# AlvinYH/Faster-VoxelPose

Hardware: AMD Instinct MI355X
Metric: frames/sec at 5-view 80x80x20 voxel (heatmaps -> 3D joints); MPJPE vs ref (mm) in mpjpe_vs_ref_mm (higher is better)
Workload: dtype f32

## Files before the change

### faster-voxelpose_amd/csrc/fvp_conv_wino.hip

```cpp
#include <hip/hip_runtime.h>

#include <algorithm>
#include <cstdio>
#include <type_traits>

#include "fvp_conv_args.h"

#ifndef FVP_WINO_ABLATE
#define FVP_WINO_ABLATE 0
#endif

namespace fvp {

typedef float f32x4 __attribute__((ext_vector_type(4)));

template <int N>
__device__ __forceinline__ void wait_vmcnt_imm() {
  static_assert(N >= 0 && N < 64, "vmcnt");
  __builtin_amdgcn_s_waitcnt(0x0f70 | (N & 15) | ((N >> 4) << 14));
}

constexpr unsigned kWinoOOB = 0x80000000u;

template <int WC, int WT, int CC, int NI, bool HAS_RES, bool RESW, int CW = 2>
__global__ void __launch_bounds__(WC * WT * 64, (WC * WT == 16 ? 4 : 2)) k_conv_wino(ConvArgs a) {
  HIP_DYNAMIC_SHARED(float, smem)
  constexpr int NWV = WC * WT;
  constexpr int NT = NWV * 64;
  static_assert(NWV == 16 || NWV == 8 || NWV == 4, "4, 8 or 16 waves");
  static_assert(CW == 1 || CW == 2, "cout blocks per wave");
  static_assert(CC == 4 || CC == 8, "chunk");
  static_assert(NI >= 1 && NI <= 4, "input DMA rounds");
  constexpr int CBW = 16 * CW * WC;
  constexpr int WCH = CC * CBW * 16;
  constexpr int WS_SZ = RESW ? 0 : WCH;
  constexpr int NW = RESW ? 0 : CC * CBW * 4 / NT;
  static_assert(RESW || (CC * CBW * 4) % NT == 0, "whole weight DMA rounds");
  constexpr int NPS = NI + NW;
  constexpr int S = CC / 4;
  constexpr int XS_SZ = NI * NT * 4;
  constexpr int BUF_SZ = XS_SZ + WS_SZ;
  constexpr bool kDiag = FVP_WINO_ABLATE != 0;
  const int t = threadIdx.x, lane = t & 63;
  const int wave = __builtin_amdgcn_readfirstlane(t >> 6);
  const int k4 = lane >> 4, l15 = lane & 15;
  const int wc = wave % WC, wt = wave / WC;
  const int W = a.W, THp = a.TH + 2, WP = W + 4;
  const int plane_sz = THp * WP;
  const int CS = a.TN * plane_sz;
  const int ablate = kDiag ? a.ablate : 0;
  const bool dma = !(ablate & 1);

  const int epi_off = 4 + 3 * BUF_SZ + (RESW ? a.cinp * CBW * 16 : 0);
  const unsigned char* const vflag = reinterpret_cast<const unsigned char*>(smem + epi_off + 3 * a.coutp);

  const int G = gridDim.x, nunits = a.nunits;
  auto next_unit = [&](int u, auto from_lds) {
    if (a.nflags > 0) {
      while (u < nunits) {
        const int pg = fdiv_nb(fdiv_nb(u, a.m_ys), a.m_ty);
        const int f = fdiv_nb(pg, a.m_vd);
        const int ok = decltype(from_lds)::value ? int(vflag[f]) : int(a.plane_valid[f]);
        if (__builtin_amdgcn_readfirstlane(ok)) break;
        u += G;
      }
    }
    return u;
  };
  using LdsFlags = std::integral_constant<bool, true>;
  using GlobalFlags = std::integral_constant<bool, false>;
  int u = next_unit(int(blockIdx.x), GlobalFlags{});
  if (u >= nunits) return;

  const int q0 = wt * 16 + l15;
  int poff;
  {
    const bool q_ok = q0 < a.TN * a.tpp;
    const int q = q_ok ? q0 : 0;
    const int tn = fdiv_nb(q, a.m_tpp), trem = q - tn * a.tpp;
    const int ty = fdiv_nb(trem, a.m_tpr), tx = trem - ty * a.tpr;
    poff = tn * plane_sz + 2 * ty * WP + 3 + 2 * tx + k4 * CS;
  }
  const int swz = (l15 >> 2) & 3;
  const int a0 = (k4 * CBW + wc * (16 * CW) + l15) * 16 + swz * 4;
  int aoff[4];
#pragma unroll
  for (int xi = 0; xi < 4; ++xi) aoff[xi] = a0 ^ (xi << 2);
  const float* const wres = smem + 4 + 3 * BUF_SZ;
  auto wchunk = [&](const float* slot, int k) { return RESW ? wres + k * WCH : slot + XS_SZ; };

  f32x4 acc[CW][16];

  const int HW = a.H * W;
  const int nchunks = a.cinp / CC;

  unsigned voff[NI];
  auto item_pos = [&](int j, int& ry, int& n, bool& inside, int& ci, int& qd) {
    const int qpr = (W >> 2) + 1;
    const int rows_per_ch = a.TN * THp;
    const int nin = CC * rows_per_ch * qpr + 1;
    int ln = lane;
    FVP_OPAQUE_V(ln);
    const int it = (wave + NWV * j) * 64 + ln;
    const int row = fdiv_nb(it, a.m_qpr);
    qd = it - row * qpr;
    ci = fdiv_nb(row, a.m_rpc);
    const int rem = row - ci * rows_per_ch;
    n = fdiv_nb(rem, a.m_thp);
    ry = rem - n * THp;
    inside = it < nin && qd > 0 && ci < CC;
  };
#pragma unroll
  for (int j = 0; j < NI; ++j) {
    int ry, n, ci, qd;
    bool inside;
    item_pos(j, ry, n, inside, ci, qd);
    voff[j] = inside ? unsigned((n * a.cin + ci) * HW + ry * W + 4 * (qd - 1)) * 4u : 0u;
    __builtin_amdgcn_sched_barrier(0);
  }
  constexpr int DCI = NT / (CBW * 4);
  const unsigned woffb = (unsigned(t / (CBW * 4)) * unsigned(a.coutp) * 16u + 4u * unsigned(t % (CBW * 4))) * 4u;
  const unsigned wdj4 = unsigned(DCI) * unsigned(a.coutp) * 64u;
  const unsigned in_step4 = unsigned(CC) * unsigned(HW) * 4u;
  const unsigned w_step4 = unsigned(CC) * unsigned(a.coutp) * 64u;
  const unsigned lds0 = FVP_LDS_BYTE_ADDRESS(smem) + 16u + unsigned(wave) * 1024u;
  i32x4 rs_in = {0, 0, 0x7ffffff0, 0x00020000}, rs_w = {0, 0, 0x7ffffff0, 0x00020000};
  auto set_base = [](i32x4& rs, const float* p) {
    const unsigned long long b = reinterpret_cast<unsigned long long>(p);
    rs[0] = __builtin_amdgcn_readfirstlane(int(unsigned(b)));
    rs[1] = __builtin_amdgcn_readfirstlane(int(unsigned(b >> 32) & 0xffffu));
  };
  int su = u, sk = 0;
  auto enter_unit = [&](int su_) {
    const KArgsPtr ka = FVP_FRESH_ARGS(a);
    const int ys = ka->ysplit, tys = ka->tiles_y;
    const int st = fdiv_nb(su_, ka->m_ys), sy = su_ - st * ys;
    const int spg = fdiv_nb(st, ka->m_ty), sty = st - spg * tys;
    const int splane0 = spg * ka->TN, sy0 = sty * ka->TH;
    const int H = ka->H, planes = ka->planes;
    set_base(rs_in, ka->src + size_t(splane0) * ka->cin * HW + sy0 * W - W);
    set_base(rs_w, ka->wts + size_t(sy) * (CBW * 16));
#pragma unroll
    for (int j = 0; j < NI; ++j) {
      int ry, n, ci, qd;
      bool inside;
      item_pos(j, ry, n, inside, ci, qd);
      const bool ok = inside && unsigned(sy0 + ry - 1) < unsigned(H) && splane0 + n < planes;
      voff[j] = (voff[j] & 0x7fffffffu) | (ok ? 0u : kWinoOOB);
      __builtin_amdgcn_sched_barrier(0);
    }
  };
  auto stage = [&](int k, int slot) {
    const unsigned la0 = lds0 + unsigned(slot) * unsigned(BUF_SZ * 4);
    const unsigned so_in = unsigned(k) * in_step4;
#pragma unroll
    for (int j = 0; j < NI; ++j) asm_buffer_load_lds16(la0 + unsigned(NWV * j) * 1024u, voff[j], rs_in, so_in);
    const unsigned so_w = unsigned(k) * w_step4;
#pragma unroll
    for (int j = 0; j < NW; ++j)
      asm_buffer_load_lds16(la0 + unsigned(XS_SZ * 4 + NWV * j * 1024), woffb, rs_w, so_w + unsigned(j) * wdj4);
  };
  enter_unit(su);
  auto stage_next = [&](int slot, auto from_lds) {
    if (su >= nunits) return false;
    stage(sk, slot);
    if (++sk == nchunks) {
      sk = 0;
      su = next_unit(su + G, from_lds);
      if (su < nunits) enter_unit(su);
    }
    return true;
  };

  float4 av[CW][4];
  float d[4][4];
  float v[4][4];
  auto fetch_a = [&](int cb, const float* wbase, int s) {
    if (kDiag && (ablate & 256)) return;
    int a0o = a0;
    if (CW == 1) FVP_OPAQUE_V(a0o);
#pragma unroll
    for (int xi = 0; xi < 4; ++xi)
      av[cb][xi] = *reinterpret_cast<const float4*>(wbase + (CW == 1 ? (a0o ^ (xi << 2)) : aoff[xi]) + (s * 4 * CBW * 16 + cb * 256));
  };
  auto fetch_d = [&](const float* base, int s, int wp) {
    const float* xs = base + poff + s * 4 * CS;
#pragma unroll
    for (int r = 0; r < 4; ++r) {
      const float* row = xs + r * wp;
      const float2 m = *reinterpret_cast<const float2*>(row + 1);
      d[r][0] = row[0];
      d[r][1] = m.x;
      d[r][2] = m.y;
      d[r][3] = row[3];
    }
  };
  auto transform = [&](float (&tr)[4][4]) {
#pragma unroll
    for (int c = 0; c < 4; ++c) {
      tr[0][c] = d[0][c] - d[2][c];
      tr[1][c] = d[1][c] + d[2][c];
      tr[2][c] = d[2][c] - d[1][c];
      tr[3][c] = d[1][c] - d[3][c];
    }
  };
  auto columns = [&](const float (&tr)[4][4]) {
#pragma unroll
    for (int xi = 0; xi < 4; ++xi) {
      v[xi][0] = tr[xi][0] - tr[xi][2];
      v[xi][1] = tr[xi][1] + tr[xi][2];
      v[xi][2] = tr[xi][2] - tr[xi][1];
      v[xi][3] = tr[xi][1] - tr[xi][3];
    }
  };
  auto mfma16 = [&](int cb, auto firstc) {
    if (kDiag && (ablate & 4)) return;
    const f32x4 z = {0.0f, 0.0f, 0.0f, 0.0f};
#pragma unroll
    for (int xi = 0; xi < 4; ++xi) {
      const float aw[4] = {av[cb][xi].x, av[cb][xi].y, av[cb][xi].z, av[cb][xi].w};
#pragma unroll
      for (int nu = 0; nu < 4; ++nu)
        acc[cb][4 * xi + nu] = __builtin_amdgcn_mfma_f32_16x16x4f32(
            aw[nu], v[xi][nu], decltype(firstc)::value ? z : acc[cb][4 * xi + nu], 0, 0, 0);
    }
  };

  if (RESW) {
    const int rounds = (a.cinp * CBW * 4) / NT;
    for (int j = 0; j < rounds; ++j)
      asm_global_load_lds16(a.wts + size_t((wave + NWV * j) * 64 + lane) * 4,
                            __builtin_amdgcn_readfirstlane(FVP_LDS_BYTE_ADDRESS(smem) +
                                                           4u * unsigned(4 + 3 * BUF_SZ + (wave + NWV * j) * 256)));
  }
  {
    float* const e = const_cast<float*>(smem) + epi_off;
    for (int i = t; i < 3 * a.coutp; i += NT) e[i] = a.epi[i];
    unsigned char* const f = const_cast<unsigned char*>(vflag);
    for (int i = t; i < a.nflags; i += NT) f[i] = a.plane_valid[i];
  }
  if (dma) {
    stage_next(0, GlobalFlags{});
    stage_next(1, GlobalFlags{});
  }
  wait_vmcnt_imm<0>();
  __syncthreads();

  int cur = 0;
  auto slot_ptr = [&](int slot) { return smem + 4 + slot * BUF_SZ; };
  fetch_a(0, wchunk(slot_ptr(0), 0), 0);
  fetch_d(slot_ptr(0), 0, WP);
  while (true) {
    auto chunk = [&](int k, auto firstc) {
      constexpr bool kFirst = decltype(firstc)::value;
      const int nxt = cur == 2 ? 0 : cur + 1;
      const int nn = nxt == 2 ? 0 : nxt + 1;
      const bool more = dma && stage_next(nn, LdsFlags{});
      const float* const cs = slot_ptr(cur);
      const float* const ns = slot_ptr(nxt);
      int wp = WP;
      FVP_OPAQUE(wp);
      if constexpr (CW == 2) {
#pragma unroll
      for (int s = 0; s < S; ++s) {
        __builtin_amdgcn_s_waitcnt(0xc07f);
        __builtin_amdgcn_sched_barrier(0);
        fetch_a(1, wchunk(cs, k), s);
        __builtin_amdgcn_sched_barrier(0);
        float tr[4][4];
        if (kDiag && (ablate & 512)) {
#pragma unroll
          for (int r = 0; r < 4; ++r)
#pragma unroll
            for (int c = 0; c < 4; ++c) v[r][c] = d[r][c];
        } else {
          transform(tr);
        }
        if (s + 1 < S) fetch_d(cs, s + 1, wp);
        __builtin_amdgcn_sched_barrier(0);
        if (!(kDiag && (ablate & 512))) columns(tr);
        if (kFirst && s == 0) mfma16(0, std::integral_constant<bool, true>{});
        else mfma16(0, std::integral_constant<bool, false>{});
        __builtin_amdgcn_sched_barrier(0);
        __builtin_amdgcn_s_waitcnt(0xc07f);
        __builtin_amdgcn_sched_barrier(0);
        if (s + 1 < S) {
          fetch_a(0, wchunk(cs, k), s + 1);
        } else {
          if (!kFirst && dma) {
            if (more) wait_vmcnt_imm<NPS>();
            else wait_vmcnt_imm<0>();
          }
          if (!(kDiag && (ablate & 128))) __builtin_amdgcn_s_barrier();
          if (k + 1 < nchunks) {
            fetch_a(0, wchunk(ns, k + 1), 0);
            fetch_d(ns, 0, wp);
          }
        }
        __builtin_amdgcn_sched_barrier(0);
        if (kFirst && s == 0) mfma16(1, std::integral_constant<bool, true>{});
        else mfma16(1, std::integral_constant<bool, false>{});
        __builtin_amdgcn_sched_barrier(0);
      }
      } else {
#pragma unroll
        for (int s = 0; s < S; ++s) {
          __builtin_amdgcn_s_waitcnt(0xc07f);
          __builtin_amdgcn_sched_barrier(0);
          {
            float tr[4][4];
            transform(tr);
            columns(tr);
          }
          __builtin_amdgcn_sched_barrier(0);
          if (kFirst && s == 0) mfma16(0, std::integral_constant<bool, true>{});
          else mfma16(0, std::integral_constant<bool, false>{});
          __builtin_amdgcn_sched_barrier(0);
          if (s + 1 < S) {
            fetch_a(0, wchunk(cs, k), s + 1);
            fetch_d(cs, s + 1, wp);
          } else {
            if (!kFirst && dma) {
              if (more) wait_vmcnt_imm<NPS>();
              else wait_vmcnt_imm<0>();
            }
            __builtin_amdgcn_s_barrier();
            if (k + 1 < nchunks) {
              fetch_a(0, wchunk(ns, k + 1), 0);
              fetch_d(ns, 0, wp);
            }
          }
          __builtin_amdgcn_sched_barrier(0);
        }
      }
      cur = nxt;
    };
    chunk(0, std::integral_constant<bool, true>{});
    for (int k = 1; k < nchunks; ++k) chunk(k, std::integral_constant<bool, false>{});

    if (!(ablate & 8)) {
      const KArgsPtr ka = FVP_FRESH_ARGS(a);
      const int ys = ka->ysplit, tys = ka->tiles_y;
      const int ut = fdiv_nb(u, ka->m_ys), uy = u - ut * ys;
      const int pg = fdiv_nb(ut, ka->m_ty), ty_i = ut - pg * tys;
      const int plane0 = pg * ka->TN, y0 = ty_i * ka->TH, co0 = uy * CBW;
      const int cout = ka->cout, coutp = ka->coutp;
      const int flags = ka->flags;
      float* const dst = ka->dst;
      const float* const res = ka->res;
      float* const pool_dst = ka->pool_dst;
      int le = lane;
      FVP_OPAQUE_V(le);
      const int k4 = le >> 4;
      const int qe = wt * 16 + (le & 15);
      const bool q_ok = qe < ka->TN * ka->tpp;
      const int qq = q_ok ? qe : 0;
      const int tn = fdiv_nb(qq, ka->m_tpp), trem = qq - tn * ka->tpp;
      const int ty = fdiv_nb(trem, ka->m_tpr), tx = trem - ty * ka->tpr;
      const bool relu = flags & FVP_EPI_RELU;
      const bool res_after = flags & FVP_EPI_RES_AFTER_RELU;
      const int plane = plane0 + tn, y = y0 + 2 * ty, x = 2 * tx;
      const bool tile_ok = q_ok && plane < ka->planes && y < ka->H;
      const unsigned ppix = unsigned((y >> 1) * (W >> 1) + tx);
      const float* const epi_s = smem + epi_off;
      const bool fast = relu && !res_after;
      unsigned HW4 = unsigned(HW) * 4u, W4 = unsigned(W) * 4u, HWq4 = unsigned(HW >> 2) * 4u;
      FVP_OPAQUE(HW4);
      FVP_OPAQUE(W4);
      FVP_OPAQUE(HWq4);
      i32x4 rs = {0, 0, 0x7ffffff0, 0x00020000};
      if (HAS_RES) set_base(rs, res + size_t(plane0) * cout * HW);
      const unsigned lco = unsigned(tn * cout + co0 + wc * (16 * CW) + 4 * k4);
      const unsigned omask = (kDiag && (ablate & 1024)) ? 0x3ffffu : 0x7fffffffu;
      const unsigned voff0 = tile_ok ? ((lco * unsigned(HW) + unsigned(y * W + x)) * 4u) & omask : kWinoOOB;
      const unsigned voffp = tile_ok ? (lco * unsigned(HW >> 2) + ppix) * 4u : kWinoOOB;
      fvp_f32x2 r0[CW][4], r1[CW][4];
      if (HAS_RES && !(kDiag && (ablate & 16))) {
        unsigned so = 0;
#pragma unroll
        for (int cb = 0; cb < CW; ++cb) {
#pragma unroll
          for (int r = 0; r < 4; ++r) {
            r0[cb][r] = asm_buffer_load_f32x2(voff0, rs, so);
            r1[cb][r] = asm_buffer_load_f32x2(voff0, rs, so + W4);
            so += HW4;
            FVP_OPAQUE(so);
          }
          so += 12u * HW4;
        }
      } else {
#pragma unroll
        for (int cb = 0; cb < CW; ++cb)
#pragma unroll
          for (int r = 0; r < 4; ++r) r0[cb][r] = r1[cb][r] = fvp_f32x2{0.f, 0.f};
      }
      float o[CW][4][2][2];
#pragma unroll
      for (int cb = 0; cb < CW; ++cb)
#pragma unroll
        for (int r = 0; r < 4; ++r) {
          float s[4][2];
#pragma unroll
          for (int xi = 0; xi < 4; ++xi) {
            const float m0 = acc[cb][4 * xi][r], m1 = acc[cb][4 * xi + 1][r], m2 = acc[cb][4 * xi + 2][r],
                        m3 = acc[cb][4 * xi + 3][r];
            s[xi][0] = (m0 + m1) + m2;
            s[xi][1] = (m1 - m2) - m3;
          }
#pragma unroll
          for (int e = 0; e < 2; ++e) {
            o[cb][r][0][e] = (s[0][e] + s[1][e]) + s[2][e];
            o[cb][r][1][e] = (s[1][e] - s[2][e]) - s[3][e];
          }
        }
      __builtin_amdgcn_sched_barrier(0);
      wait_vmcnt_imm<0>();
      __builtin_amdgcn_sched_barrier(0);
      auto finalize = [&](auto fastc) {
        constexpr bool kFast = decltype(fastc)::value;
        set_base(rs, dst + size_t(plane0) * cout * HW);
        float pm[CW][4];
        unsigned sso = 0;
#pragma unroll
        for (int cb = 0; cb < CW; ++cb) {
          const int co4 = co0 + wc * (16 * CW) + cb * 16 + 4 * k4;
          f32x4 bn[3];
#pragma unroll
          for (int i = 0; i < 3; ++i) bn[i] = *reinterpret_cast<const f32x4*>(epi_s + i * coutp + co4);
#pragma unroll
          for (int r = 0; r < 4; ++r) {
            const float b = bn[0][r], sc = bn[1][r], sh = bn[2][r];
            const float rr[2][2] = {{r0[cb][r].x, r0[cb][r].y}, {r1[cb][r].x, r1[cb][r].y}};
            float vv[2][2];
#pragma unroll
            for (int i = 0; i < 2; ++i)
#pragma unroll
              for (int e = 0; e < 2; ++e) {
                float xv = bn_affine(o[cb][r][i][e], b, sc, sh);
                if (HAS_RES && (kFast || !res_after)) xv += rr[i][e];
                if (kFast || relu) xv = fmaxf(xv, 0.0f);
                if (HAS_RES && !kFast && res_after) xv += rr[i][e];
                vv[i][e] = xv;
              }
            pm[cb][r] = fmaxf(fmaxf(vv[0][0], vv[0][1]), fmaxf(vv[1][0], vv[1][1]));
            if (kDiag && (ablate & 32) && vv[0][0] != 1.2345e-30f) { sso += HW4; continue; }
            asm_buffer_store_f32x2(fvp_f32x2{vv[0][0], vv[0][1]}, voff0, rs, sso);
            asm_buffer_store_f32x2(fvp_f32x2{vv[1][0], vv[1][1]}, voff0, rs, sso + W4);
            sso += HW4;
            FVP_OPAQUE(sso);
          }
          sso += 12u * HW4;
        }
        if (pool_dst && !(kDiag && (ablate & 32))) {
          set_base(rs, pool_dst + size_t(plane0) * cout * (HW >> 2));
#pragma unroll
          for (int cb = 0; cb < CW; ++cb)
#pragma unroll
            for (int r = 0; r < 4; ++r)
              asm_buffer_store_f32(pm[cb][r], voffp, rs, unsigned(cb * 16 + r) * HWq4);
        }
      };
      if (fast) finalize(std::integral_constant<bool, true>{});
      else finalize(std::integral_constant<bool, false>{});
    } else {
      wait_vmcnt_imm<0>();
    }
    u = next_unit(u + G, LdsFlags{});
    if (u >= nunits) break;
    fetch_a(0, wchunk(slot_ptr(cur), 0), 0);
    fetch_d(slot_ptr(cur), 0, WP);
  }
}

__global__ void __launch_bounds__(256)
k_pack_wino(const float* __restrict__ w, int cin, int cout, int cinp, int coutp, float* __restrict__ dst) {
  const int i = blockIdx.x * 256 + threadIdx.x;
  if (i >= cinp * coutp) return;
  const int co = i % coutp, ci = i / coutp;
  float g[3][3];
#pragma unroll
  for (int ky = 0; ky < 3; ++ky)
#pragma unroll
    for (int kx = 0; kx < 3; ++kx)
      g[ky][kx] = (co < cout && ci < cin) ? w[(size_t(co) * cin + ci) * 9 + ky * 3 + kx] : 0.0f;
  float gg[4][3];
#pragma unroll
  for (int kx = 0; kx < 3; ++kx) {
    const float e = g[0][kx] + g[2][kx];
    gg[0][kx] = g[0][kx];
    gg[1][kx] = 0.5f * (e + g[1][kx]);
    gg[2][kx] = 0.5f * (e - g[1][kx]);
    gg[3][kx] = g[2][kx];
  }
  float* out = dst + size_t(i) * 16;
  const int swz = (co >> 2) & 3;
#pragma unroll
  for (int xi = 0; xi < 4; ++xi) {
    const float e = gg[xi][0] + gg[xi][2];
    float* o = out + 4 * (xi ^ swz);
    o[0] = gg[xi][0];
    o[1] = 0.5f * (e + gg[xi][1]);
    o[2] = 0.5f * (e - gg[xi][1]);
    o[3] = gg[xi][2];
  }
}

static const size_t kWinoLdsBudget = env_size("FVP_WINO_LDS_KB", 152) * 1024;
static const int kWinoGeneric = int(env_size("FVP_WINO_GENERIC", 0));
constexpr int kWinoMaskedMinW = 40;
static const int kWinoWC1 = int(env_size("FVP_WINO_WC1", 0));
static const int kWinoHalf = int(env_size("FVP_WINO_HALF", 0));
static const int kWinoNoResW = int(env_size("FVP_WINO_NO_RESW", 0));
static const int kWinoAblate = int(env_size("FVP_CONV_ABLATE", 0));
#ifndef FVP_WINO_W16_DEFAULT
#define FVP_WINO_W16_DEFAULT 0
#endif

int persistent_workgroups() {
  static int n = 0;
  if (!n) {
    int dev = 0, cus = 0;
    if (hipGetDevice(&dev) != hipSuccess ||
        hipDeviceGetAttribute(&cus, hipDeviceAttributeMultiprocessorCount, dev) != hipSuccess || cus <= 0)
      cus = 256;
    n = int(env_size("FVP_WINO_WGS", size_t(cus)));
  }
  return n;
}

static bool wino_tiling(int h, int w, int cinp, int coutp, int* WC, int* WT, int* TN, int* TR, bool half = false) {
  if (h < 2 || (h & 1) || w < 8 || (w & 3) || (coutp != 32 && coutp % 64 != 0) || cinp % 4 != 0) return false;
  if ((w & (w - 1)) && w < kWinoMaskedMinW && !kWinoGeneric) return false;
  *WC = (coutp == 32 || kWinoWC1 || half) ? 1 : 2;
  *WT = (half ? 4 : 8) / *WC;
  const int tpr = w / 2, TT = 16 * *WT, rows = h / 2;
  if (tpr > TT) return false;
  if (rows * tpr >= TT) {
    *TN = 1;
    *TR = TT / tpr;
  } else {
    *TN = TT / (rows * tpr);
    *TR = rows;
  }
  return true;
}

bool wino_shape_ok(int h, int w, int cinp, int coutp) {
  int WC, WT, TN, TR;
  return wino_tiling(h, w, cinp, coutp, &WC, &WT, &TN, &TR);
}

template <int WC, int WT, int CC, int NI, bool RES, bool RESW, int CW = 2>
static int launch_wino3(const ConvArgs& a, dim3 grid, size_t lds, hipStream_t s) {
  static LdsOptIn optin;
  auto k = &k_conv_wino<WC, WT, CC, NI, RES, RESW, CW>;
  if (int e = lds_opt_in(optin, reinterpret_cast<const void*>(k), 160 * 1024)) return e;
  hipLaunchKernelGGL(k, grid, dim3(WC * WT * 64), lds, s, a);
  return launch_status();
}
template <int WC, int WT, int CC, bool RESW, int CW = 2>
static int launch_wino2(const ConvArgs& a, dim3 grid, size_t lds, hipStream_t s) {
  const bool res = a.flags & FVP_EPI_RES;
  switch (a.wino_ni) {
    case 1: return res ? launch_wino3<WC, WT, CC, 1, true, RESW, CW>(a, grid, lds, s) : launch_wino3<WC, WT, CC, 1, false, RESW, CW>(a, grid, lds, s);
    case 2: return res ? launch_wino3<WC, WT, CC, 2, true, RESW, CW>(a, grid, lds, s) : launch_wino3<WC, WT, CC, 2, false, RESW, CW>(a, grid, lds, s);
    case 3: return res ? launch_wino3<WC, WT, CC, 3, true, RESW, CW>(a, grid, lds, s) : launch_wino3<WC, WT, CC, 3, false, RESW, CW>(a, grid, lds, s);
    case 4: return res ? launch_wino3<WC, WT, CC, 4, true, RESW, CW>(a, grid, lds, s) : launch_wino3<WC, WT, CC, 4, false, RESW, CW>(a, grid, lds, s);
  }
  return FVP_ELIMIT;
}
#if FVP_DIAG
template <int WC, int WT, bool RESW>
static int launch_wino16(const ConvArgs& a, dim3 grid, size_t lds, hipStream_t s) {
  const bool res = a.flags & FVP_EPI_RES;
  if (a.wino_ni == 1)
    return res ? launch_wino3<WC, WT, 8, 1, true, RESW, 1>(a, grid, lds, s) : launch_wino3<WC, WT, 8, 1, false, RESW, 1>(a, grid, lds, s);
  if (a.wino_ni == 2)
    return res ? launch_wino3<WC, WT, 8, 2, true, RESW, 1>(a, grid, lds, s) : launch_wino3<WC, WT, 8, 2, false, RESW, 1>(a, grid, lds, s);
  return FVP_ELIMIT;
}
#endif
template <int WC, int WT>
static int launch_wino(const ConvArgs& a, dim3 grid, size_t lds, hipStream_t s, bool resw) {
  if (WC == 1 && WT == 8 && resw && a.CC == 8) return launch_wino2<1, 8, 8, true>(a, grid, lds, s);
  if (a.CC == 8) return launch_wino2<WC, WT, 8, false>(a, grid, lds, s);
  return launch_wino2<WC, WT, 4, false>(a, grid, lds, s);
}

int wino_plan_and_launch(const FvpConvOp& op, ConvArgs a, const float* params, int planes, hipStream_t s) {
  int WC, WT, TN, TR;
  if (conv_form(op, planes, a.pool_dst != nullptr, a.w2 != nullptr) != ConvForm::Wino) return FVP_EINVAL;
  if (!wino_tiling(op.h, op.w, op.cinp, op.coutp, &WC, &WT, &TN, &TR, kWinoHalf == 1)) return FVP_EINVAL;
  if (kWinoHalf == 0) {
    const long units = long(ceil_div(op.h / 2, TR)) * ceil_div(planes, TN) * (op.coutp / (32 * WC));
    int wc, wt, tn, tr;
    if (units < persistent_workgroups() && wino_tiling(op.h, op.w, op.cinp, op.coutp, &wc, &wt, &tn, &tr, true)) {
      WC = wc; WT = wt; TN = tn; TR = tr;
    }
  }
#if FVP_DIAG
  static const int kW16 = int(env_size("FVP_WINO_W16", FVP_WINO_W16_DEFAULT));
#else
  constexpr int kW16 = 0;
#endif
  const bool w16 = kW16 && WC * WT == 8 && op.cinp % 8 == 0;
  static const int kQuarter = int(env_size("FVP_WINO_QUARTER", 1));
  bool quarter = false;
  if (kQuarter && !w16 && WC * WT == 4 && op.cinp % 4 == 0) {
    const long units_half = long(ceil_div(op.h / 2, TR)) * ceil_div(planes, TN) * (op.coutp / 32);
    quarter = units_half * (kQuarter == 2 ? 1 : 2) < persistent_workgroups();
  }
  const int CW = (w16 || quarter) ? 1 : 2;
  if (w16) WC *= 2;
  a.ablate = kWinoAblate;
  a.wts = params + op.wino_off;
  a.TN = TN;
  a.TH = 2 * TR;
  a.TW = op.w;
  a.tiles_x = 1;
  a.tiles_y = ceil_div(op.h / 2, TR);
  a.tpp = TR * (op.w / 2);
  a.m_tpp = make_magic(a.tpp);
  a.tpr = op.w / 2;
  a.m_tpr = make_magic(a.tpr);
  a.vec = a.dma = 1;
  a.zeros = params;
  const int CBW = 16 * CW * WC;
  const size_t resw_bytes = size_t(op.cinp) * CBW * 64;
  const size_t budget = WC * WT == 4 ? std::min<size_t>(kWinoLdsBudget, 78 * 1024) : kWinoLdsBudget;
  const size_t epi_bytes = size_t(3) * op.coutp * 4;
  a.nflags = (a.plane_valid && TN == 1) ? ceil_div(planes, a.valid_div) : 0;
  a.m_vd = make_magic(a.valid_div);
  const size_t flag_bytes = size_t(a.nflags + 15) & ~size_t(15);
  bool resw = CBW == 32 && WT == 8 && op.coutp == 32 && op.cinp % 8 == 0 && resw_bytes <= 64 * 1024 && !kWinoNoResW;
  auto slot_bytes = [&](int cc, int* ni, bool rw) {
    const size_t quads = size_t(cc) * TN * (a.TH + 2) * (op.w / 4 + 1) + 1;
    const size_t per_round = size_t(WC) * WT * 64;
    *ni = int((quads + per_round - 1) / per_round);
    return size_t(*ni) * per_round * 16 + (rw ? 0 : size_t(cc) * CBW * 64);
  };
  const size_t fixed = 64 + epi_bytes + flag_bytes;
  int CC = op.cinp % 8 == 0 ? 8 : 4, ni = 0;
  size_t slot = slot_bytes(CC, &ni, resw);
  if (resw && (3 * slot + resw_bytes + fixed > budget || ni > 4)) {
    resw = false;
    slot = slot_bytes(CC, &ni, false);
  }
  if (CC == 8 && !resw && (3 * slot + fixed > budget || ni > 4)) {
    CC = 4;
    slot = slot_bytes(CC, &ni, false);
  }
  if (3 * slot + (resw ? resw_bytes : 0) + fixed > budget || ni > 4) return FVP_ELIMIT;
  a.CC = CC;
  a.wino_ni = ni;
  if (!buf_dma_range_ok(TN, op.cin, op.h, op.w, double(op.cinp) * op.coutp * 16)) return FVP_ELIMIT;
  if ((double(TN) + 1.0) * op.cout * op.h * op.w * 4.0 >= 2147483648.0) return FVP_ELIMIT;
  a.m_qpr = make_magic(op.w / 4 + 1);
  a.m_rpc = make_magic(TN * (a.TH + 2));
  a.m_thp = make_magic(a.TH + 2);
  const size_t lds = 16 + 3 * slot + (resw ? resw_bytes : 0) + epi_bytes + flag_bytes;
  a.ysplit = op.coutp / CBW;
  a.nunits = a.tiles_y * ceil_div(planes, TN) * a.ysplit;
  a.m_ys = make_magic(a.ysplit);
  a.m_ty = make_magic(a.tiles_y);
  static const int kBalanced = int(env_size("FVP_WINO_BALANCED", 0));
  const int slots = persistent_workgroups() * (WC * WT == 4 ? 2 : 1);
  dim3 grid(kBalanced ? ceil_div(a.nunits, ceil_div(a.nunits, slots)) : std::min(a.nunits, slots), 1, 1);
  ProfScope ps(a.nunits < slots ? FVP_K_CONV_WINO_SMALL : FVP_K_CONV_WINO, s, 2.0 * op.cin * op.cout * 9.0 * op.h * op.w * planes, 1,
               prof_level() >= 2);
#if FVP_DIAG
  if (w16) {
    if (CC != 8 || ni > 2) return FVP_ELIMIT;
    if (CBW == 32) return resw ? launch_wino16<2, 8, true>(a, grid, lds, s) : launch_wino16<2, 8, false>(a, grid, lds, s);
    return launch_wino16<4, 4, false>(a, grid, lds, s);
  }
#endif
  if (quarter) return a.CC == 8 ? launch_wino2<1, 4, 8, false, 1>(a, grid, lds, s) : launch_wino2<1, 4, 4, false, 1>(a, grid, lds, s);
  if (WC * WT == 4) return launch_wino<1, 4>(a, grid, lds, s, false);
  return WC == 1 ? launch_wino<1, 8>(a, grid, lds, s, resw) : launch_wino<2, 4>(a, grid, lds, s, false);
}

int wino_pack(const float* weight, const FvpConvOp& op, float* params, hipStream_t s) {
  hipLaunchKernelGGL(k_pack_wino, dim3(ceil_div(op.cinp * op.coutp, 256)), dim3(256), 0, s, weight, op.cin, op.cout,
                     op.cinp, op.coutp, params + op.wino_off);
  return launch_status();
}

}
```

Before: 3017.

## Prefetch residual tile before final MFMA block to overlap epilogue loads

For residual Winograd conv variants with two cout blocks per wave, the second MFMA group of each chunk moves to the start of the next chunk. The last group is deferred until after the main loop, and the residual global loads are issued before it so their latency hides behind the final MFMAs instead of stalling the epilogue. This reshuffles the MFMA schedule across chunk boundaries and keeps residual registers live longer, which raises register pressure and could hurt occupancy. A compile-time macro enables it by default.

```diff
diff --git a/faster-voxelpose_amd/csrc/fvp_conv_wino.hip b/faster-voxelpose_amd/csrc/fvp_conv_wino.hip
--- a/faster-voxelpose_amd/csrc/fvp_conv_wino.hip
+++ b/faster-voxelpose_amd/csrc/fvp_conv_wino.hip
@@ -6,6 +6,9 @@
 
 #include "fvp_conv_args.h"
 
+#ifndef FVP_WINO_RES_PF
+#define FVP_WINO_RES_PF 1
+#endif
 #ifndef FVP_WINO_ABLATE
 #define FVP_WINO_ABLATE 0
 #endif
@@ -250,9 +253,54 @@
   auto slot_ptr = [&](int slot) { return smem + 4 + slot * BUF_SZ; };
   fetch_a(0, wchunk(slot_ptr(0), 0), 0);
   fetch_d(slot_ptr(0), 0, WP);
+  constexpr bool kTail = FVP_WINO_RES_PF && HAS_RES && CW == 2;
+  const bool res_pf = kTail && !(kDiag && (ablate & 16));
+  fvp_f32x2 r0[CW][4], r1[CW][4];
+  i32x4 rs_res = {0, 0, 0x7ffffff0, 0x00020000};
+  unsigned voff_res = kWinoOOB;
+  auto res_setup = [&]() {
+    const KArgsPtr ka = FVP_FRESH_ARGS(a);
+    const int ys = ka->ysplit, tys = ka->tiles_y;
+    const int ut = fdiv_nb(u, ka->m_ys), uy = u - ut * ys;
+    const int pg = fdiv_nb(ut, ka->m_ty), ty_i = ut - pg * tys;
+    const int plane0 = pg * ka->TN, y0 = ty_i * ka->TH, co0 = uy * CBW;
+    const int cout = ka->cout;
+    int le = lane;
+    FVP_OPAQUE_V(le);
+    const int qe = wt * 16 + (le & 15);
+    const bool q_ok = qe < ka->TN * ka->tpp;
+    const int qq = q_ok ? qe : 0;
+    const int tn = fdiv_nb(qq, ka->m_tpp), trem = qq - tn * ka->tpp;
+    const int ty = fdiv_nb(trem, ka->m_tpr), tx = trem - ty * ka->tpr;
+    const int plane = plane0 + tn, y = y0 + 2 * ty, x = 2 * tx;
+    const bool tile_ok = q_ok && plane < ka->planes && y < ka->H;
+    const unsigned lco = unsigned(tn * cout + co0 + wc * (16 * CW) + 4 * (le >> 4));
+    const unsigned omask = (kDiag && (ablate & 1024)) ? 0x3ffffu : 0x7fffffffu;
+    voff_res = tile_ok ? ((lco * unsigned(HW) + unsigned(y * W + x)) * 4u) & omask : kWinoOOB;
+    set_base(rs_res, ka->res + size_t(plane0) * cout * HW);
+  };
+  auto res_load = [&](int cb) {
+    unsigned HW4 = unsigned(HW) * 4u, W4 = unsigned(W) * 4u;
+    FVP_OPAQUE(HW4);
+    FVP_OPAQUE(W4);
+    unsigned so = unsigned(cb * 16) * HW4;
+#pragma unroll
+    for (int r = 0; r < 4; ++r) {
+      r0[cb][r] = asm_buffer_load_f32x2(voff_res, rs_res, so);
+      r1[cb][r] = asm_buffer_load_f32x2(voff_res, rs_res, so + W4);
+      so += HW4;
+      FVP_OPAQUE(so);
+    }
+  };
+
   while (true) {
     auto chunk = [&](int k, auto firstc) {
       constexpr bool kFirst = decltype(firstc)::value;
+      const bool has_next = k + 1 < nchunks;
+      if constexpr (kTail && !kFirst) {
+        mfma16(1, std::integral_constant<bool, false>{});
+        __builtin_amdgcn_sched_barrier(0);
+      }
       const int nxt = cur == 2 ? 0 : cur + 1;
       const int nn = nxt == 2 ? 0 : nxt + 1;
       const bool more = dma && stage_next(nn, LdsFlags{});
@@ -292,14 +340,17 @@
             else wait_vmcnt_imm<0>();
           }
           if (!(kDiag && (ablate & 128))) __builtin_amdgcn_s_barrier();
-          if (k + 1 < nchunks) {
+          if (has_next) {
             fetch_a(0, wchunk(ns, k + 1), 0);
             fetch_d(ns, 0, wp);
           }
         }
         __builtin_amdgcn_sched_barrier(0);
-        if (kFirst && s == 0) mfma16(1, std::integral_constant<bool, true>{});
-        else mfma16(1, std::integral_constant<bool, false>{});
+        if (kTail && s + 1 == S) {
+        } else {
+          if (kFirst && s == 0) mfma16(1, std::integral_constant<bool, true>{});
+          else mfma16(1, std::integral_constant<bool, false>{});
+        }
         __builtin_amdgcn_sched_barrier(0);
       }
       } else {
@@ -325,7 +376,7 @@
               else wait_vmcnt_imm<0>();
             }
             __builtin_amdgcn_s_barrier();
-            if (k + 1 < nchunks) {
+            if (has_next) {
               fetch_a(0, wchunk(ns, k + 1), 0);
               fetch_d(ns, 0, wp);
             }
@@ -335,8 +386,24 @@
       }
       cur = nxt;
     };
+    if constexpr (kTail && S == 1) {
+#pragma unroll
+      for (int i = 0; i < 16; ++i) acc[1][i] = f32x4{0.0f, 0.0f, 0.0f, 0.0f};
+    }
     chunk(0, std::integral_constant<bool, true>{});
     for (int k = 1; k < nchunks; ++k) chunk(k, std::integral_constant<bool, false>{});
+    if constexpr (kTail) {
+      if (res_pf) {
+        res_setup();
+        res_load(0);
+        if (!RESW) res_load(1);
+      }
+      __builtin_amdgcn_sched_barrier(0);
+      mfma16(1, std::integral_constant<bool, false>{});
+      __builtin_amdgcn_sched_barrier(0);
+      if (RESW && res_pf) res_load(1);
+      __builtin_amdgcn_sched_barrier(0);
+    }
 
     if (!(ablate & 8)) {
       const KArgsPtr ka = FVP_FRESH_ARGS(a);
@@ -374,8 +441,8 @@
       const unsigned omask = (kDiag && (ablate & 1024)) ? 0x3ffffu : 0x7fffffffu;
       const unsigned voff0 = tile_ok ? ((lco * unsigned(HW) + unsigned(y * W + x)) * 4u) & omask : kWinoOOB;
       const unsigned voffp = tile_ok ? (lco * unsigned(HW >> 2) + ppix) * 4u : kWinoOOB;
-      fvp_f32x2 r0[CW][4], r1[CW][4];
-      if (HAS_RES && !(kDiag && (ablate & 16))) {
+      if (res_pf) {
+      } else if (HAS_RES && !(kDiag && (ablate & 16))) {
         unsigned so = 0;
 #pragma unroll
         for (int cb = 0; cb < CW; ++cb) {
@@ -443,9 +510,10 @@
                 vv[i][e] = xv;
               }
             pm[cb][r] = fmaxf(fmaxf(vv[0][0], vv[0][1]), fmaxf(vv[1][0], vv[1][1]));
-            if (kDiag && (ablate & 32) && vv[0][0] != 1.2345e-30f) { sso += HW4; continue; }
-            asm_buffer_store_f32x2(fvp_f32x2{vv[0][0], vv[0][1]}, voff0, rs, sso);
-            asm_buffer_store_f32x2(fvp_f32x2{vv[1][0], vv[1][1]}, voff0, rs, sso + W4);
+            if (!(kDiag && (ablate & 32) && vv[0][0] != 1.2345e-30f)) {
+              asm_buffer_store_f32x2(fvp_f32x2{vv[0][0], vv[0][1]}, voff0, rs, sso);
+              asm_buffer_store_f32x2(fvp_f32x2{vv[1][0], vv[1][1]}, voff0, rs, sso + W4);
+            }
             sso += HW4;
             FVP_OPAQUE(sso);
           }
```

Measured after the change: 3019, median of 2. About the same (+0.1%).
